# ai4ce/V2X-Sim

Measured on AMD Instinct MI355X. Metric: BEV frames/sec, V2VNet 5-agent detection (256x256 BEV), higher is better.
Workload: dtype bf16

## Files before the change

### v2x-sim_amd/csrc/api.hip

```cpp
#include "common.h"

static thread_local char g_err[512] = "";

void v2x_set_error(const char *fmt, ...) {
    va_list ap;
    va_start(ap, fmt);
    vsnprintf(g_err, sizeof(g_err), fmt, ap);
    va_end(ap);
}

extern "C" __attribute__((weak)) int v2x_probe_build_marker;
extern "C" int v2x_abi_version(void) { return &v2x_probe_build_marker != nullptr ? -V2X_AMD_ABI_VERSION : V2X_AMD_ABI_VERSION; }

#include <atomic>
#include <mutex>
#include <strings.h>
namespace {
struct TuneEntry { const char *name; int def; };
const TuneEntry kTune[V2X_TUNE_COUNT] = {
    {"STREAM_WAVES", 8}, {"STREAM_G", 1}, {"STREAM_WT", 1}, {"STORE_X4", 1}, {"STREAM_PERSIST", 1}, {"STREAM_WIDE", 1},
    {"WIDE3", 1}, {"HALO_PP", 1}, {"VOXELIZE_LDS", 1}, {"WARP_LDS", 2}, {"S2_G", 1}, {"GRU_XCD_WALK", 1}, {"HALO_XCD", 1}, {"WGRAD_TR", 1}, {"BN_PARTIAL_T", 1}, {"WGRAD_REDUCE4", 1}, {"CONV1X1", 1},
};
std::atomic<int> g_tune[V2X_TUNE_COUNT];
std::once_flag g_tune_once;
void tune_init() {
    for (int i = 0; i < V2X_TUNE_COUNT; ++i) {
        char env[64];
        snprintf(env, sizeof(env), "V2X_%s", kTune[i].name);
        const char *e = getenv(env);
        g_tune[i].store((e && *e) ? atoi(e) : kTune[i].def, std::memory_order_relaxed);
    }
}
int tune_find(const char *name) {
    if (!name) return -1;
    if (strncasecmp(name, "V2X_", 4) == 0) name += 4;
    for (int i = 0; i < V2X_TUNE_COUNT; ++i)
        if (strcasecmp(name, kTune[i].name) == 0) return i;
    return -1;
}
}

int v2x_tune(int id) {
    std::call_once(g_tune_once, tune_init);
    return g_tune[id].load(std::memory_order_relaxed);
}
extern "C" int v2x_tuning_set(const char *name, int value) {
    const int i = tune_find(name);
    V2X_REQUIRE(i >= 0, "v2x_tuning_set: unknown switch '%s'", name ? name : "(null)");
    std::call_once(g_tune_once, tune_init);
    g_tune[i].store(value, std::memory_order_relaxed);
    return V2X_OK;
}
extern "C" int v2x_tuning_get(const char *name, int *value) {
    const int i = tune_find(name);
// ... 6 lines not shown
```

### v2x-sim_amd/csrc/common.h

```cpp
#pragma once
#include <hip/hip_runtime.h>
#include <stdint.h>
#include <stdio.h>
#include <stdarg.h>

#include "../../include/v2x_amd.h"

typedef __attribute__((ext_vector_type(8))) __bf16 bf16x8_t;
typedef __attribute__((ext_vector_type(4))) float f32x4_t;
typedef __attribute__((ext_vector_type(16))) float f32x16_t;

void v2x_set_error(const char *fmt, ...);

enum v2x_tune_id {
    V2X_TUNE_STREAM_WAVES,
    V2X_TUNE_STREAM_G,
    V2X_TUNE_STREAM_WT,
    V2X_TUNE_STORE_X4,
    V2X_TUNE_STREAM_PERSIST,
    V2X_TUNE_STREAM_WIDE,
    V2X_TUNE_WIDE3,
    V2X_TUNE_HALO_PP,
    V2X_TUNE_VOXELIZE_LDS,
    V2X_TUNE_WARP_LDS,
    V2X_TUNE_S2_G,
    V2X_TUNE_GRU_XCD_WALK,
    V2X_TUNE_HALO_XCD,
    V2X_TUNE_WGRAD_TR,
    V2X_TUNE_BN_PARTIAL_T,
    V2X_TUNE_WGRAD_REDUCE4,
    V2X_TUNE_CONV1X1,
    V2X_TUNE_COUNT
};
int v2x_tune(int id);

#define V2X_REQUIRE(cond, ...)            \
    do {                                  \
        if (!(cond)) {                    \
            v2x_set_error(__VA_ARGS__);   \
            return V2X_EINVAL;            \
        }                                 \
    } while (0)

#define V2X_CHECK_LAUNCH(name)                                                   \
    do {                                                                         \
        hipError_t e_ = hipGetLastError();                                       \
        if (e_ != hipSuccess) {                                                  \
            v2x_set_error("%s: launch failed: %s", name, hipGetErrorString(e_)); \
            return V2X_EIO;                                                      \
        }                                                                        \
    } while (0)

#define V2X_MAX_DEVICES 32
struct v2x_once_per_device { bool done[V2X_MAX_DEVICES]; };
static inline bool v2x_first_use_on_device(v2x_once_per_device &o) {
    int dev = 0;
    if (hipGetDevice(&dev) != hipSuccess || dev < 0 || dev >= V2X_MAX_DEVICES) return true;
    if (o.done[dev]) return false;
    o.done[dev] = true;
    return true;
}

__device__ __forceinline__ uint16_t f32_to_bf16_rne(float f) {
    uint32_t u = __float_as_uint(f);
// ... 55 lines not shown
```

### v2x-sim_amd/csrc/conv_halo.hip

```cpp
#include "common.h"
#include <cstdlib>

static __device__ __attribute__((aligned(64))) unsigned int g_zero_page_h[16];

typedef const __attribute__((address_space(1))) void *gptr_t;
typedef __attribute__((address_space(3))) void *lptr_t;

__device__ __forceinline__ void glds16h(const void *g, char *lds_wave_base) {
    __builtin_amdgcn_global_load_lds((gptr_t)g, (lptr_t)lds_wave_base, 16, 0, 0);
}

struct HaloArgs {
    const uint16_t *in0;
    const uint16_t *in1;
    const uint32_t *bits;
    int zbits;
    int N, H, W;
    const uint16_t *w;
    const float *scale, *shift;
    int relu;
    void *out;
    int out_cstride, out_coff;
    const uint16_t *w2;
    const float *scale2, *shift2;
// ... 486 lines not shown
                    if constexpr (EPI2 == 2) {
                        const bool second = a.split > 0 && co >= a.split;
                        float *dst = second ? reinterpret_cast<float *>(a.out2) + pix * a.out2_cstride + (co - a.split)
                                            : reinterpret_cast<float *>(a.out) + pix * a.out_cstride + a.out_coff + co;
                        *reinterpret_cast<float4 *>(dst) = make_float4(v0, v1, v2, v3);
                    } else {
                        uint2 o;
                        o.x = pack_bf16x2(v0, v1);
                        o.y = pack_bf16x2(v2, v3);
                        uint16_t *dst = reinterpret_cast<uint16_t *>(a.out) + pix * a.out_cstride + a.out_coff + co;
                        *reinterpret_cast<uint2 *>(dst) = o;
                    }
                }
            }
        }
        if constexpr (DB) {
            cur ^= 1;
        } else {
            __builtin_amdgcn_s_barrier();
        }
    }
}

template <int C0, int C1, int COUT, int COUT2, int EPI2>
__global__ __launch_bounds__(256) __attribute__((amdgpu_waves_per_eu((C0 == 0 && C1 == 64 && COUT2 == 64) ? 1 : 2, 2))) void conv3x3_halo_kernel(const HaloArgs a) {
    conv3x3_halo_body<C0, C1, COUT, COUT2, EPI2, true>(a);
}

template <int C0, int C1, int COUT, int COUT2, int EPI2, bool BITS>
__global__ __launch_bounds__(256) __attribute__((amdgpu_waves_per_eu(4, 4))) void conv3x3_halo_sb_kernel(const HaloArgs a) {
    conv3x3_halo_body<C0, C1, COUT, COUT2, EPI2, false, BITS>(a);
}

template <int C0, int C1, int COUT, int COUT2 = 0>
__global__ __launch_bounds__(512) __attribute__((amdgpu_waves_per_eu(2, 2))) void conv3x3_halo_pp_kernel(const HaloArgs a) {
    constexpr int SPP0 = C0 / 8, SPP1 = C1 / 8;
    constexpr int NS1 = round64(PH * PW * SPP1);
    constexpr int NS0 = C0 ? round64(PH0 * PW0 * SPP0) : 0;
    constexpr int PATCH_BYTES = (NS0 + NS1) * 16;
    constexpr int KSLOTS = 9 * (SPP0 + SPP1);
    constexpr int W_BYTES = KSLOTS * COUT * 16;
    constexpr int TCO = COUT / 16;
    static_assert(C0 % 32 == 0 && C1 % 32 == 0 && (TCO == 2 || TCO == 4), "ping-pong form: 32 or 64 output channels");
    static_assert(W_BYTES % 1024 == 0, "weights are moved 1 KiB per wave instruction");
    constexpr int TCO2 = COUT2 / 16;
    static_assert(COUT2 == 0 || (COUT2 == 64 && COUT == 64), "chained 1x1: 64 -> 64 (conv1_2 -> conv3d_1)");
    constexpr int N_STORES = (COUT2 ? TCO2 : TCO) * 4;

    extern __shared__ __attribute__((aligned(16))) char smem[];
    const uint32_t relu_floor = a.relu ? 0u : 0x80008000u;
    char *s_w = smem;
    char *s_patch = smem + W_BYTES;
    float *s_ss = reinterpret_cast<float *>(smem + W_BYTES + 2 * PATCH_BYTES);
    for (int i = threadIdx.x; i < COUT; i += 512) {
        s_ss[i] = a.scale[i];
        s_ss[COUT + i] = a.shift[i];
    }
    if constexpr (COUT2 > 0) {
        for (int i = threadIdx.x; i < COUT2; i += 512) {
            s_ss[2 * COUT + i] = a.scale2[i];
            s_ss[2 * COUT + COUT2 + i] = a.shift2[i];
        }
    }

    const int tid = threadIdx.x;
    const int lane = tid & 63;
    const int wave = __builtin_amdgcn_readfirstlane(tid >> 6);
    const int grp = wave >> 2, wv = wave & 3;
// ... 279 lines not shown
                    uint32_t ox[2], oy[2];
#pragma unroll
                    for (int h = 0; h < 2; ++h) {
                        ox[h] = v2x_relu_bf16x2_floor(pack_bf16x2(acc[i + h][f][0] * sc[h].x + sf[h].x, acc[i + h][f][1] * sc[h].y + sf[h].y), relu_floor);
                        oy[h] = v2x_relu_bf16x2_floor(pack_bf16x2(acc[i + h][f][2] * sc[h].z + sf[h].z, acc[i + h][f][3] * sc[h].w + sf[h].w), relu_floor);
                    }
                    v2x_store_pair_x4(reinterpret_cast<uint16_t *>(a.out) + ((size_t)(n * a.H + y) * a.W + x) * a.out_cstride + a.out_coff + i * 16 + fq * 4, fq,
                                      ox[0], oy[0], ox[1], oy[1]);
                }
            }
            return;
        }
#pragma unroll
        for (int i = 0; i < TCO; ++i) {
            const int co = i * 16 + fq * 4;
            const float4 sc = *reinterpret_cast<const float4 *>(ss + co);
            const float4 sf = *reinterpret_cast<const float4 *>(ss + COUT + co);
#pragma unroll
            for (int f = 0; f < 4; ++f) {
                const int y = y0 + 2 * wv + (f >> 1), x = x0 + (f & 1) * 16 + fj;
                float v0 = acc[i][f][0] * sc.x + sf.x, v1 = acc[i][f][1] * sc.y + sf.y;
                float v2 = acc[i][f][2] * sc.z + sf.z, v3 = acc[i][f][3] * sc.w + sf.w;
                uint2 o;
                o.x = pack_bf16x2(v0, v1);
                o.y = pack_bf16x2(v2, v3);
                o.x = v2x_relu_bf16x2_floor(o.x, relu_floor);
                o.y = v2x_relu_bf16x2_floor(o.y, relu_floor);
                uint16_t *dst = reinterpret_cast<uint16_t *>(a.out) + ((size_t)(n * a.H + y) * a.W + x) * a.out_cstride + a.out_coff + co;
                *reinterpret_cast<uint2 *>(dst) = o;
            }
        }
    };

    const int n_pairs = a.n_tiles >> 1;
    const v2x_tile_walk walk = v2x_xcd_tile_walk(n_pairs, a.xcd_walk);
    const int K = walk.first < walk.end ? (walk.end - walk.first + walk.step - 1) / walk.step : 0;
    auto tile_of = [&](int k) { return 2 * (walk.first + k * walk.step) + grp; };

    if (grp == 0) load_patch(tile_of(0));
    __syncthreads();

    for (int i = 0; i <= 2 * K; ++i) {
        if ((i & 1) == grp) {
            if ((i >> 1) < K) compute();
        } else {
            const int m = (i - grp - 1) / 2;
            if (m + 1 < K) load_patch(tile_of(m + 1));
            if (m >= 0) {
                epilogue(tile_of(m));
                if constexpr (N_STORES == 8) {
                    if (a.x4) asm volatile("s_waitcnt vmcnt(4)" ::: "memory");
                    else asm volatile("s_waitcnt vmcnt(8)" ::: "memory");
                } else {
                    if (a.x4) asm volatile("s_waitcnt vmcnt(8)" ::: "memory");
                    else asm volatile("s_waitcnt vmcnt(16)" ::: "memory");
                }
            } else {
                asm volatile("s_waitcnt vmcnt(0)" ::: "memory");
            }
        }
        __builtin_amdgcn_sched_barrier(0);
        __builtin_amdgcn_s_barrier();
        __builtin_amdgcn_sched_barrier(0);
    }
    static_assert(N_STORES == 8 || N_STORES == 16, "the counted waits above know 8 or 16 stores per tile and wave");
}

template <int C0, int C1, int COUT, int COUT2 = 0>
static int launch_halo_pp(const HaloArgs &a, hipStream_t s) {
    constexpr int NS1 = round64(PH * PW * (C1 / 8));
    constexpr int NS0 = C0 ? round64(PH0 * PW0 * (C0 / 8)) : 0;
    constexpr int smem = 9 * (C0 + C1) / 8 * COUT * 16 + 2 * (NS0 + NS1) * 16 + 2 * COUT * 4 + 2 * COUT2 * 4;
    static_assert(smem <= 160 * 1024, "LDS budget");
    static v2x_once_per_device attr_once;
    auto kern = &conv3x3_halo_pp_kernel<C0, C1, COUT, COUT2>;
    if (v2x_first_use_on_device(attr_once)) {
        (void)hipFuncSetAttribute(reinterpret_cast<const void *>(kern), hipFuncAttributeMaxDynamicSharedMemorySize, smem);
    }
    int grid = 256;
    if (grid > a.n_tiles / 2) grid = a.n_tiles / 2;
    hipLaunchKernelGGL(kern, dim3(grid), dim3(512), smem, s, a);
    V2X_CHECK_LAUNCH("conv3x3_halo_pp_kernel");
    return V2X_OK;
}

constexpr int PWH = PW / 2;

template <int C0, int C1, int COUT>
__global__ __launch_bounds__(512) __attribute__((amdgpu_waves_per_eu(2, 2))) void conv3x3_halo_ppc_kernel(const HaloArgs a) {
    constexpr int SPP0 = C0 / 8, SPP1 = C1 / 8;
    constexpr int NS1 = round64(2 * PH * PWH * SPP1);
    constexpr int NS0 = round64(PH0 * PW0 * SPP0);
    constexpr int PATCH_BYTES = (NS0 + NS1) * 16;
    constexpr int W_UP_BYTES = 16 * SPP0 * COUT * 16;
    constexpr int W_BYTES = W_UP_BYTES + 9 * SPP1 * COUT * 16;
    constexpr int TCO = COUT / 16;
    constexpr int KC0 = C0 / 32, KC1 = C1 / 32;
    static_assert(C0 % 32 == 0 && C1 % 32 == 0 && C0 > 0 && C1 > 0 && TCO == 2, "parity-class form: two sources, 32 output channels");
    static_assert(W_BYTES % 1024 == 0, "weights are moved 1 KiB per wave instruction");
    constexpr int N_STORES = TCO * 4;

    extern __shared__ __attribute__((aligned(16))) char smem[];
    const uint32_t relu_floor = a.relu ? 0u : 0x80008000u;
    char *s_w = smem;
    char *s_patch = smem + W_BYTES;
    float *s_ss = reinterpret_cast<float *>(smem + W_BYTES + 2 * PATCH_BYTES);
    for (int i = threadIdx.x; i < COUT; i += 512) {
        s_ss[i] = a.scale[i];
        s_ss[COUT + i] = a.shift[i];
    }

    const int tid = threadIdx.x;
    const int lane = tid & 63;
    const int wave = __builtin_amdgcn_readfirstlane(tid >> 6);
    const int grp = wave >> 2, wv = wave & 3;
// ... 277 lines not shown
            const double slack = fmax(1e-3, 4e-7 / (t * (1.0 - t)));
            a.det_margin = (float)fmin(log(t / (1.0 - t)) - slack, 16.0);
        }
    }
    a.det_cap = d->det_cap;
    {
        const int cmax = d->C1 ? (d->C0 > d->C1 ? d->C0 : d->C1) : d->C0;
        if ((long long)(PH * d->W + PW) * cmax >= (1 << 20)) return 1;
    }
    a.tiles_x = d->W / TW;
    a.tiles_y = d->H / TH;
    a.n_tiles = d->N * a.tiles_x * a.tiles_y;
    const int co2 = d->Cout2 > 0 ? (d->Cout2 + 15) / 16 * 16 : 0;
    const int e2 = d->Cout2 > 0 ? (d->epilogue == V2X_EPI_DET ? 3 : (d->epilogue == V2X_EPI_F32 ? 2 : 1)) : 0;
#define HALO_CASE(c0, c1, co, c2, ep) \
    if (C0 == c0 && C1 == c1 && d->Cout == co && co2 == c2 && e2 == ep) return launch_halo<c0, c1, co, c2, ep>(a, s);
    if (C0 == 0 && C1 == 32 && d->Cout == 32 && co2 == 0 && e2 == 0)
        return d->in_format == 1 ? launch_halo_sb<0, 32, 32, 0, 0, true>(a, s) : launch_halo_sb<0, 32, 32, 0, 0, false>(a, s);
    if (d->in_format == 1) return 1;
    if (d->w_layout == 3) {
        if (C0 == 64 && C1 == 32 && d->Cout == 32 && co2 == 0 && e2 == 0) return launch_halo_ppc<64, 32, 32>(a, s);
        return 1;
    }
    if (C0 == 64 && C1 == 32 && d->Cout == 32 && co2 == 0 && e2 == 0 && a.n_tiles >= 2 && a.n_tiles % 2 == 0) {
        if (v2x_tune(V2X_TUNE_HALO_PP) != 0) return launch_halo_pp<64, 32, 32>(a, s);
    }
    HALO_CASE(64, 32, 32, 0, 0)
    if (C0 == 0 && C1 == 64 && d->Cout == 64 && co2 == 0 && e2 == 0 && a.n_tiles >= 2 && a.n_tiles % 2 == 0) {
        if (v2x_tune(V2X_TUNE_HALO_PP) != 0) return launch_halo_pp<0, 64, 64>(a, s);
    }
    HALO_CASE(0, 64, 64, 0, 0)
    if (C0 == 0 && C1 == 64 && d->Cout == 64 && co2 == 64 && e2 == 1 && d->Cout2 == 64 && a.n_tiles >= 2 && a.n_tiles % 2 == 0 &&
        d->split == 0)
        return launch_halo_pp<0, 64, 64, 64>(a, s);
    HALO_CASE(0, 64, 64, 64, 1)
    HALO_CASE(0, 64, 32, 0, 0)
    HALO_CASE(0, 32, 64, 0, 0)
    HALO_CASE(0, 32, 64, 48, 2)
    HALO_CASE(0, 32, 32, 16, 2)
    if (e2 == 3) {
        if (!(C0 == 0 && C1 == 32 && d->Cout == 64 && d->Cout2 == 64 && d->det_counts && d->out && d->out2 && d->det_cap > 0 &&
              d->det_cap <= 4096 && (long long)d->H * d->W * 6 < (1 << 20)))
            return 1;
        return launch_halo<0, 32, 64, 64, 3>(a, s);
    }
#undef HALO_CASE
    return 1;
}
```

### v2x-sim_amd/csrc/conv_stream.hip

```cpp
#include "conv_stream.h"
#include <cstdlib>
#include <type_traits>



#ifndef V2X_STREAM_PSWZ_BUILD
#define V2X_STREAM_PSWZ_BUILD 1
#endif
#define PSWZ(pc) (((pc) >> V2X_STREAM_PSWZ_BUILD) & 3)
#ifndef V2X_STREAM_LSS_BUILD
#define V2X_STREAM_LSS_BUILD 1
#endif

template <int N>
__device__ __forceinline__ void wait_vmcnt() {
    asm volatile("s_waitcnt vmcnt(%0)" ::"n"(N) : "memory");
}

template <int BCO>
constexpr int chain_lds_bytes() { return BCO * BCO * 2 + 2 * BCO * 4; }

template <int BCO, int NT>
__device__ __forceinline__ void stage_chain(const StreamArgs &a, char *cl) {
    constexpr int NKS = BCO / 32;
// ... 424 lines not shown
            f32x4_t g[3];
#pragma unroll
            for (int q = 0; q < 3; ++q) g[q] = (f32x4_t){0.f, 0.f, 0.f, 0.f};
            for (int sp = 0; sp < ksplit; ++sp)
#pragma unroll
                for (int q = 0; q < 3; ++q) g[q] += *reinterpret_cast<const f32x4_t *>(ws + ((size_t)sp * npix + pix) * w_rows + row + 16 * q);
            float h[4];
#pragma unroll
            for (int r = 0; r < 4; ++r) {
                const float4 b = reinterpret_cast<const float4 *>(scale)[c + r];
                h[r] = v2x_gru_h0(g[0][r], g[1][r], g[2][r], b);
            }
            uint2 o;
            o.x = pack_bf16x2(h[0], h[1]);
            o.y = pack_bf16x2(h[2], h[3]);
            *reinterpret_cast<uint2 *>(out + pix * out_cstride + out_coff + c) = o;
        } else {
            f32x4_t v = (f32x4_t){0.f, 0.f, 0.f, 0.f};
            for (int sp = 0; sp < ksplit; ++sp) v += *reinterpret_cast<const f32x4_t *>(ws + ((size_t)sp * npix + pix) * w_rows + c);
            const float4 sc = *reinterpret_cast<const float4 *>(scale + c), sf = *reinterpret_cast<const float4 *>(shift + c);
            uint2 o;
            o.x = pack_bf16x2(v[0] * sc.x + sf.x, v[1] * sc.y + sf.y);
            o.y = pack_bf16x2(v[2] * sc.z + sf.z, v[3] * sc.w + sf.w);
            if (relu) {
                o.x = v2x_relu_bf16x2(o.x);
                o.y = v2x_relu_bf16x2(o.y);
            }
            *reinterpret_cast<uint2 *>(out + pix * out_cstride + out_coff + c) = o;
        }
    }
}


template <int BCO, int EPI>
__global__ __launch_bounds__(512) __attribute__((amdgpu_waves_per_eu(2, 2))) void conv3x3_stream8_kernel(const StreamArgs a) {
    constexpr bool PERSIST = (EPI != SEPI_CHAIN);
    constexpr int TH = 16, TW = 32;
    constexpr int PW = TW + 2, PH = TH + 2, PW0 = TW / 2 + 2, PH0 = TH / 2 + 2;
    constexpr int TCO = BCO / 16;
    constexpr int W_PIECES = BCO / 16;
    constexpr int SLICE_BYTES = BCO * 64;
    constexpr int N_ST = (EPI == SEPI_GRU) ? (TCO / 3) * 4 : TCO * 4;
    static_assert(PH * PW * 4 <= (PATCH8_PIECES - 1) * 64, "patch must leave the last piece as padding");
    static_assert(W_PIECES <= 8, "at most one weight DMA per wave per step");
    static_assert(4 + N_ST <= 63, "vmcnt is a 6-bit counter");

    extern __shared__ __attribute__((aligned(16))) char smem[];
    char *s_ring = smem;
    char *s_patch = smem + RING * SLICE_BYTES;
    char *s_dummy = s_patch + (PATCH8_PIECES - 1) * 1024;

    const int tid = threadIdx.x;
    const int lane = tid & 63;
    const int wave = __builtin_amdgcn_readfirstlane(tid >> 6);
    const int grp = wave >> 2, wv = wave & 3;
    const int fj = lane & 15, fq = lane >> 4;

    const int nwg = gridDim.x;
    int bid = blockIdx.x;
    {
        const int q = nwg >> 3, r = nwg & 7, xcd = bid & 7, i = bid >> 3;
        bid = (xcd < r ? xcd * (q + 1) : r * (q + 1) + (xcd - r) * q) + i;
    }
    const int n_tiles = a.n_px_tiles * a.n_co_tiles;
    const int co_tile = bid % a.n_co_tiles;
    const int txy = a.tiles_x * a.tiles_y;

    const int nc0 = a.C0 >> 5, nchunks = (a.C0 + a.C1) >> 5;
    const int S = nchunks * 9;
    const uint16_t *wbase = a.w + (size_t)co_tile * nchunks * 9 * (BCO * 32);
    const void *zero_page = a.w + (size_t)a.n_co_tiles * nchunks * 9 * (BCO * 32);
    char *s_chain = smem + RING * SLICE_BYTES + 2 * PATCH8_BYTES;
    if constexpr (EPI == SEPI_CHAIN) stage_chain<BCO, 512>(a, s_chain);

    auto tile_coords = [&](int t, int &n, int &y0, int &x0) {
        const int px_tile = t / a.n_co_tiles;
        n = px_tile / txy;
        const int trem = px_tile - n * txy;
        const int ty = trem / a.tiles_x;
        y0 = ty * TH;
        x0 = (trem - ty * a.tiles_x) * TW;
    };
    auto desc = [&](int n, int y0, int x0, int t, bool hf) -> int {
        const int L = (wave + 8 * t) * 64 + lane;
        const int pix = L >> 2, phys = L & 3;
        if (!hf) {
            const int pr = pix / PW, pc = pix - pr * PW;
            const int y = y0 - 1 + pr, x = x0 - 1 + pc;
            const bool ok = pix < PH * PW && (unsigned)y < (unsigned)a.H && (unsigned)x < (unsigned)a.W;
            return ok ? ((((n * a.H + y) * a.W + x) << 5) | ((phys ^ PSWZ(pc)) << 3)) : -1;
        }
        const int Hs = a.H >> 1, Ws = a.W >> 1;
        const int pr = pix / PW0, pc = pix - pr * PW0;
        const int y = (y0 >> 1) - 1 + pr, x = (x0 >> 1) - 1 + pc;
        const bool ok = pix < PH0 * PW0 && (unsigned)y < (unsigned)Hs && (unsigned)x < (unsigned)Ws;
        return ok ? ((((n * Hs + y) * Ws + x) << 5) | ((phys ^ PSWZ(pc)) << 3)) : -1;
    };

    int frow[4], ct[4][3];
#pragma unroll
    for (int f = 0; f < 4; ++f) frow[f] = 8 * grp + 2 * wv + (f >> 1);
    auto build_ct = [&](bool hf) {
#pragma unroll
        for (int f = 0; f < 4; ++f) {
            const int col = (f & 1) * 16 + fj;
#pragma unroll
            for (int kx = 0; kx < 3; ++kx) {
                const int pc = hf ? (((col + kx - 1) >> 1) + 1) : (col + kx);
                ct[f][kx] = ((pc << 2) + (fq ^ PSWZ(pc))) * 16;
            }
        }
    };

    const bool has_w = wave < W_PIECES;
    const uint16_t *wsrc = wbase + lane * 8 + wave * 512;
    auto issue_dummy = [&]() { glds16s(zero_page, s_dummy); };
    auto issue_slice = [&](int slice, int slot, bool real) {
// ... 88 lines not shown
#pragma unroll
                    for (int i = 0; i < TCO; ++i)
                        fa[i] = *reinterpret_cast<const bf16x8_t *>(ws + (fq * BCO + i * 16 + fj) * 16);
                    if (relaxed > 0) {
                        wait_vmcnt<4 + N_ST>();
                        --relaxed;
                    } else {
                        wait_vmcnt<4>();
                    }
                    asm volatile("s_waitcnt lgkmcnt(0)" ::: "memory");
                    __builtin_amdgcn_sched_barrier(0);
                    __builtin_amdgcn_s_barrier();
                    __builtin_amdgcn_sched_barrier(0);
#pragma unroll
                    for (int i = 0; i < TCO; ++i)
#pragma unroll
                        for (int f = 0; f < 4; ++f)
                            acc[i][f] = __builtin_amdgcn_mfma_f32_16x16x32_bf16(fa[i], fb[f], acc[i][f], 0, 0, 0);
                    __builtin_amdgcn_sched_barrier(0);
                    __builtin_amdgcn_s_barrier();
                    __builtin_amdgcn_sched_barrier(0);
                }
            }
        }
        stream_epilogue<BCO, TW, EPI, 4, EPI == SEPI_CHAIN, true, EPI == SEPI_CHAIN>(a, acc, co_tile, n, y0, x0, frow, fj, fq, s_chain, nullptr, 0, a.x4 != 0);
        if (!has_next) break;
        tile = next;
        n = nn;
        y0 = ny0;
        x0 = nx0;
        relaxed = 2;
    }
    if (grp == 0) __builtin_amdgcn_s_barrier();
}

int v2x_conv_stream_pc_launch(const StreamArgs &a, hipStream_t s);

int v2x_num_cus() {
    static int n[V2X_MAX_DEVICES] = {0};
    int dev = 0, v = 0;
    if (hipGetDevice(&dev) != hipSuccess || dev < 0 || dev >= V2X_MAX_DEVICES) return 256;
    if (n[dev] == 0)
        n[dev] = (hipDeviceGetAttribute(&v, hipDeviceAttributeMultiprocessorCount, dev) == hipSuccess && v > 0) ? v : 256;
    return n[dev];
}

#define V2X_STREAM8G_ISSUE_DMAS \
                if (grp == 1) { \
                    const int ahead = st + 2; \
                    const int wslot = slot == 0 ? 2 : slot - 1; \
                    if (ahead < S3) nw = issue_weights(ahead, wslot, wv, 4); \
                    else if (has_next && ahead - S3 < S3) nw = issue_weights(ahead - S3, wslot, wv, 4); \
                } else if (fill && kx < 2) { \
                    const int npieces = hfn ? (PH0 * PW0 * 4 + 63) / 64 : PATCH8_PIECES; \
_Pragma("unroll") \
                    for (int t = 0; t < 5; ++t) { \
                        const int tt = kx * 5 + t; \
                        if (wv + 4 * tt >= npieces) break; \
                        int d = pd[0]; \
_Pragma("unroll") \
                        for (int u = 1; u < 10; ++u) d = (tt == u) ? pd[u] : d; \
                        issue_piece(d, kcn, tt, (gc + 1) & 1); \
                    } \
                }
template <int BCO, int EPI, bool WT = false>
__global__ __launch_bounds__(512) __attribute__((amdgpu_waves_per_eu(2, 2))) void conv3x3_stream8g_kernel(const StreamArgs a) {
// ... 280 lines not shown
        constexpr bool LSS = V2X_STREAM_LSS_BUILD != 0 && EPI != SEPI_GRU;
        if constexpr (WT)
            stream_epilogue<BCO / 2, TW, EPI, 8, false, true, true>(a, acc, co_tile * 2 + coh, n, y0, x0, frow, fj, fq, nullptr,
                                                                    LSS ? (lds_cf_t *)s_ss + coh * (EPI == SEPI_GRU ? 4 * (BCO / 6) : BCO / 2) : (lds_cf_t *)nullptr, BCO, a.x4 != 0);
        else stream_epilogue<BCO, TW, EPI, 4, false, true, true>(a, acc, co_tile, n, y0, x0, frow, fj, fq, nullptr, LSS ? (lds_cf_t *)s_ss : (lds_cf_t *)nullptr, BCO, a.x4 != 0);
        if (!has_next) break;
        tile = next;
        n = nn;
        y0 = ny0;
        x0 = nx0;
        relaxed = true;
    }
    if (grp == 0) __builtin_amdgcn_s_barrier();
}

template <int BCO, int EPI, bool WT = false>
static int launch_stream8g(const StreamArgs &a, hipStream_t s) {
    constexpr int smem = 3 * 3 * BCO * 64 + 2 * PATCH8_BYTES + 1024;
    static_assert(smem <= 160 * 1024, "LDS budget");
    static v2x_once_per_device attr_once;
    auto kern = &conv3x3_stream8g_kernel<BCO, EPI, WT>;
    if (v2x_first_use_on_device(attr_once)) {
        (void)hipFuncSetAttribute(reinterpret_cast<const void *>(kern), hipFuncAttributeMaxDynamicSharedMemorySize, smem);
    }
    const int n_tiles = a.n_px_tiles * a.n_co_tiles;
    int grid = n_tiles;
    int g = v2x_num_cus() / a.n_co_tiles * a.n_co_tiles;
    if (g > 0 && g < n_tiles) grid = g;
    hipLaunchKernelGGL(kern, dim3(grid), dim3(512), smem, s, a);
    V2X_CHECK_LAUNCH("conv3x3_stream8g_kernel");
    return V2X_OK;
}

template <int BCO, int EPI>
static int launch_stream8(const StreamArgs &a, hipStream_t s) {
    constexpr int smem = RING * BCO * 64 + 2 * PATCH8_BYTES + (EPI == SEPI_CHAIN ? chain_lds_bytes<BCO>() : 0);
    static v2x_once_per_device attr_once;
    auto kern = &conv3x3_stream8_kernel<BCO, EPI>;
    if (v2x_first_use_on_device(attr_once)) {
        (void)hipFuncSetAttribute(reinterpret_cast<const void *>(kern), hipFuncAttributeMaxDynamicSharedMemorySize, smem);
    }
    const int n_tiles = a.n_px_tiles * a.n_co_tiles;
    int grid = n_tiles;
    if (v2x_tune(V2X_TUNE_STREAM_PERSIST) != 0) {
        int g = v2x_num_cus() / a.n_co_tiles * a.n_co_tiles;
        if (EPI != SEPI_CHAIN && g > 0 && g < n_tiles && ((a.C0 + a.C1) >> 5) >= 2) grid = g;
    }
    hipLaunchKernelGGL(kern, dim3(grid), dim3(512), smem, s, a);
    V2X_CHECK_LAUNCH("conv3x3_stream8_kernel");
    return V2X_OK;
}

constexpr int WPATCH_PIECES = 39;
constexpr int WPATCH_BYTES = WPATCH_PIECES * 1024;

template <int BCO, int EPI>
__global__ __launch_bounds__(256) __attribute__((amdgpu_waves_per_eu(2, 2))) void conv3x3_wide_kernel(const StreamArgs a) {
    constexpr int TH = 16, TW = 32, NF = 8;
    constexpr int PW = TW + 2, PH = TH + 2, PW0 = TW / 2 + 2, PH0 = TH / 2 + 2;
    constexpr int TCO = BCO / 16;
    constexpr int SLICE_BYTES = BCO * 64;
    constexpr int PPW = (WPATCH_PIECES + 3) / 4;
    static_assert(BCO == 64, "wide form: one 64-row channel tile (1 weight DMA per wave and step)");
    static_assert(PH * PW * 4 <= WPATCH_PIECES * 64, "patch must fit its buffer");

    extern __shared__ __attribute__((aligned(16))) char smem[];
    char *s_ring = smem;
    char *s_patch = smem + RING * SLICE_BYTES;

    const int tid = threadIdx.x;
    const int lane = tid & 63;
    const int wave = __builtin_amdgcn_readfirstlane(tid >> 6);
    const int fj = lane & 15, fq = lane >> 4;

    int bid = blockIdx.x;
    {
        const int nwg = gridDim.x, q = nwg >> 3, r = nwg & 7, xcd = bid & 7, i = bid >> 3;
        bid = (xcd < r ? xcd * (q + 1) : r * (q + 1) + (xcd - r) * q) + i;
    }
    const int co_tile = bid % a.n_co_tiles;
    const int px_tile = bid / a.n_co_tiles;
    const int txy = a.tiles_x * a.tiles_y;
// ... 421 lines not shown
            if (d->W % 64 != 0) return 1;
            a.tiles_x = d->W / 64;
            a.n_co_tiles = 1;
        } else {
            a.n_co_tiles = d->Cout / 128;
        }
        a.n_px_tiles = d->N * a.tiles_x * a.tiles_y;
        return v2x_conv_stream_pc_launch(a, s);
    }
    const bool chain = d->Cout2 > 0;
    if (d->splitk > 1) {
        const int nchunks = (d->C0 + d->C1) >> 5;
        const int per = (nchunks + d->splitk - 1) / d->splitk;
        if (chain || !d->splitk_ws || d->splitk > nchunks || per * (d->splitk - 1) >= nchunks || (rows != 128 && rows != 96 && rows != 64)) return 1;
        if (d->epilogue == V2X_EPI_GRU) return t16 ? launch_stream_splitk<96, 16, 16, SEPI_GRU>(a, s) : launch_stream_splitk<96, 8, 32, SEPI_GRU>(a, s);
        if (rows == 128) return t16 ? launch_stream_splitk<128, 16, 16, SEPI_BF16>(a, s) : launch_stream_splitk<128, 8, 32, SEPI_BF16>(a, s);
        return t16 ? launch_stream_splitk<64, 16, 16, SEPI_BF16>(a, s) : launch_stream_splitk<64, 8, 32, SEPI_BF16>(a, s);
    }
    if (chain) {
        if ((d->Cout != 64 && d->Cout != 128) || d->Cout2 != d->Cout || d->w_rows != d->Cout || d->epilogue != V2X_EPI_BF16 ||
            !d->weight2 || !d->scale2 || !d->shift2)
            return 1;
    }
    const bool few_chain_tiles = chain && (long long)d->N * (d->H / 16) * (d->W / 32) * 4 < 3ll * v2x_num_cus();
    if (!t16 && d->H % 16 == 0 && (rows == 128 || rows == 96) && !few_chain_tiles) {
        if (v2x_tune(V2X_TUNE_STREAM_WAVES) != 4) {
            a.tiles_y = d->H / 16;
            a.n_px_tiles = d->N * a.tiles_x * a.tiles_y;
            const bool grouped = v2x_tune(V2X_TUNE_STREAM_G) != 0 && !chain && a.n_co_tiles <= v2x_num_cus();
            const int wt = v2x_tune(V2X_TUNE_STREAM_WT);
            if (grouped && wt >= 1 && d->epilogue != V2X_EPI_GRU) return launch_stream8g<128, SEPI_BF16, true>(a, s);
            if (grouped && wt >= 2 && d->epilogue == V2X_EPI_GRU) return launch_stream8g<96, SEPI_GRU, true>(a, s);
            if (d->epilogue == V2X_EPI_GRU) return grouped ? launch_stream8g<96, SEPI_GRU>(a, s) : launch_stream8<96, SEPI_GRU>(a, s);
            if (chain) return launch_stream8<128, SEPI_CHAIN>(a, s);
            return grouped ? launch_stream8g<128, SEPI_BF16>(a, s) : launch_stream8<128, SEPI_BF16>(a, s);
        }
    }
    if (!t16 && d->H % 16 == 0 && rows == 64 && d->epilogue == V2X_EPI_BF16 && ((d->C0 + d->C1) >> 5) >= 2) {
        if (v2x_tune(V2X_TUNE_STREAM_WIDE) != 0) {
            a.tiles_y = d->H / 16;
            a.n_px_tiles = d->N * a.tiles_x * a.tiles_y;
            if (!chain && ((d->C0 + d->C1) >> 5) >= 3 && v2x_tune(V2X_TUNE_WIDE3) != 0) return launch_wide3<64>(a, s);
            return chain ? launch_wide<64, SEPI_CHAIN>(a, s) : launch_wide<64, SEPI_BF16>(a, s);
        }
    }
    if (chain) {
        if (d->Cout == 128) return t16 ? launch_stream<128, 16, 16, SEPI_CHAIN>(a, s) : launch_stream<128, 8, 32, SEPI_CHAIN>(a, s);
        return t16 ? launch_stream<64, 16, 16, SEPI_CHAIN>(a, s) : launch_stream<64, 8, 32, SEPI_CHAIN>(a, s);
    }
    if (d->epilogue == V2X_EPI_GRU) return t16 ? launch_stream<96, 16, 16, SEPI_GRU>(a, s) : launch_stream<96, 8, 32, SEPI_GRU>(a, s);
    if (rows == 128) return t16 ? launch_stream<128, 16, 16, SEPI_BF16>(a, s) : launch_stream<128, 8, 32, SEPI_BF16>(a, s);
    return t16 ? launch_stream<64, 16, 16, SEPI_BF16>(a, s) : launch_stream<64, 8, 32, SEPI_BF16>(a, s);
}
```

### v2x-sim_amd/v2x_sim_amd/ops.py

```python
import ctypes as C

import torch

from . import _lib, tuning
from ._lib import ConvDesc, V2X_EPI_BF16, V2X_EPI_F32, V2X_EPI_GRU, V2X_FUSE_MAX, V2X_FUSE_MEAN, V2X_FUSE_WSUM


from . import _launch
from ._launch import _Prof, _dev, _dev_opt, _stream


import threading as _threading

_latency = _threading.local()


class latency_dispatch:

    def __init__(self, target=0):
        self.target = target

    def __enter__(self):
        _latency.depth = getattr(_latency, "depth", 0) + 1
        self.prev, _latency.target = getattr(_latency, "target", 0), self.target
# ... 24 lines not shown


def conv_kernel_name(pc, H=0, W=0, bits=False, N=0):
    if pc.w_layout == 2 and pc.stride == 2:
        if pc.Cout == 64 and pc.C0 == 32:
            return "conv3x3_s2_resident_kernel<64>"
        rows = 128 if pc.Cout % 128 == 0 else 64
        s2g = tuning.get("S2_G")
        if rows == 128 and pc.C0 >= 64 and s2g != 0:
            Ho, Wo = H // 2, W // 2
            g32 = Ho % 8 == 0 and Wo % 32 == 0
            g16 = not g32 and Ho % 16 == 0 and Wo % 16 == 0
            tiles = N * (Ho * Wo // 256) * (pc.Cout // 128)
            if (g32 or g16) and not (latency_launches() and tiles < 4 * torch.cuda.get_device_properties(0).multi_processor_count):
                return "conv3x3_s2g_kernel<%s>" % ("8, 32" if g32 else "16, 16")
        if not (H % 8 == 0 and W % 64 == 0):
            return "conv3x3_s2_stream_kernel<%d, 8, 16>" % rows
        return "conv3x3_s2_stream_kernel<%d, 4, 32>" % rows
    if pc.w_layout == 2:
        rows = _lib.load().v2x_conv_stream_tile_rows(pc.Cout, pc.epilogue)
        th, tw = (8, 32) if W % 32 == 0 else (16, 16)
        epi = 2 if pc.epilogue == V2X_EPI_GRU else (1 if pc.Cout2 else 0)
        if W % 32 == 0 and H % 16 == 0 and rows == 64 and pc.epilogue == V2X_EPI_BF16 and (pc.C0 + pc.C1) >= 64 \
                and tuning.get("STREAM_WIDE") != 0:
            if epi == 0 and (pc.C0 + pc.C1) >= 96 and tuning.get("WIDE3") != 0:
                return "conv3x3_wide3_kernel<64>"
            return "conv3x3_wide_kernel<64, %d>" % epi
        if W % 32 == 0 and H % 16 == 0 and rows in (96, 128) \
                and tuning.get("STREAM_WAVES") != 4:
            if epi != 1 and tuning.get("STREAM_G") != 0:
                wt = tuning.get("STREAM_WT")
                tiled = (wt >= 1 and epi == 0) or (wt >= 2 and epi == 2)
                return "conv3x3_stream8g_kernel<%d, %d, %s>" % (rows, epi, "true" if tiled else "false")
            return "conv3x3_stream8_kernel<%d, %d>" % (rows, epi)
        return "conv3x3_stream_kernel<%d, %d, %d, %d, false>" % (rows, th, tw, epi)
    if pc.w_layout == 4:
        return "conv3x3_stream8q_kernel" if pc.Cout == 64 else "conv3x3_stream8p_kernel"
    if pc.w_layout == 3:
        return "conv3x3_halo_ppc_kernel<%d, %d, %d>" % (pc.C0, pc.C1, pc.Cout)
    if pc.w_layout == 1:
        c0, c1 = (pc.C0, pc.C1) if pc.C1 else (0, pc.C0)
        co2 = (pc.Cout2 + 15) // 16 * 16 if pc.Cout2 else 0
        e2 = 0 if not pc.Cout2 else (2 if pc.epilogue == V2X_EPI_F32 else 1)
        if (c0, c1, pc.Cout, co2) == (0, 32, 32, 0):
            return "conv3x3_halo_sb_kernel<0, 32, 32, 0, 0, %s>" % ("true" if bits else "false")
        if (c0, c1, pc.Cout, co2, e2) == (0, 64, 64, 64, 1):
            return "conv3x3_halo_pp_kernel<0, 64, 64, 64>"
        if (c0, c1, pc.Cout, co2) in ((64, 32, 32, 0), (0, 64, 64, 0)) and tuning.get("HALO_PP") != 0:
            return "conv3x3_halo_pp_kernel<%d, %d, %d, 0>" % (c0, c1, pc.Cout)
        return "conv3x3_halo_kernel<%d, %d, %d, %d, %d>" % (c0, c1, pc.Cout, co2, e2)
    if (pc.ksize == 1 and pc.stride == 1 and not pc.C1 and not pc.Cout2 and pc.epilogue in (V2X_EPI_BF16, V2X_EPI_F32) and pc.C0 % 32 == 0 and pc.C0 <= 128
            and pc.C0 // 32 != 3 and 4 <= pc.Cout <= 128 and pc.Cout % 4 == 0 and (pc.Cout + 15) // 16 in (1, 2, 3, 4, 6, 8) and tuning.get("CONV1X1") != 0):
        ks, ct = pc.C0 // 32, (pc.Cout + 15) // 16
        return "conv1x1_stream_kernel<%d, %d, %s, %d>" % (ks, ct, "true" if pc.epilogue == V2X_EPI_F32 else "false", 2 if ks * ct >= 16 else 4)
    rows = _lib.load().v2x_conv_tile_rows(pc.Cout, pc.epilogue)
    return "conv_igemm_kernel<%d, %d, %d, %d, %d>" % (_CONV_TILES[rows] + (pc.epilogue,))


class VoxelGrid:

    def __init__(self, voxel_size=(0.25, 0.25, 0.4), area_extents=((-32.0, 32.0), (-32.0, 32.0), (-3.0, 2.0))):
        import math
        self.voxel = tuple(float(v) for v in voxel_size)
        self.extents = tuple((float(lo), float(hi)) for lo, hi in area_extents)
        self.dims = tuple(int(math.ceil(hi / v) - 1 - math.floor(lo / v) + 1)
                          for (lo, hi), v in zip(self.extents, self.voxel))
        self._ext = (C.c_double * 6)(*[x for lohi in self.extents for x in lohi])
        self._vox = (C.c_double * 3)(*self.voxel)
        self._dims = (C.c_int32 * 3)(*self.dims)


def voxelize_bits(points, n_pts, grid, out=None):
    lib = _lib.load()
    if points.dim() != 3:
        raise ValueError("points must be (n_clouds, max_pts, stride)")
    n, mp, st = points.shape
    if tuple(n_pts.shape) != (n,):
        raise ValueError("n_pts must hold one count per cloud: expected shape (%d,), got %s" % (n, tuple(n_pts.shape)))
    X, Y, Z = grid.dims
# ... 480 lines not shown
```

### v2x-sim_amd/v2x_sim_amd/tuning.py

```python
import ctypes as C
import os

_HOST_DEFAULTS = {"CONV_PAIR": 1, "TRAIN_HIP": 1, "TRAIN_GRAPH": 1, "TRAIN_HIP_CONV": 0, "SMALL_BATCH": 2, "WARP_HIP": 1, "WARP_XCD": 1, "SEG_FUSE": 1, "TRAIN_PACK_BATCH": 1, "TRAIN_LOSS_HIP": 1, "TRAIN_GATES_HIP": 1, "PARITY_CLASS": 3, "TAIL_FUSE": 1, "TRAIN_HEAD_PACK": 1, "TRAIN_BN_BIAS_ZERO": 1, "TRAIN_UPCAT_CONV": 1, "TRAIN_SPLITK": 480, "TRAIN_V2V_NHWC": 1, "TRAIN_ADAM_HIP": 1, "SPLITK_TARGET": 320}
LIBRARY_SWITCHES = ("STREAM_WAVES", "STREAM_G", "STREAM_WT", "STORE_X4", "STREAM_PERSIST", "STREAM_WIDE", "WIDE3", "HALO_PP",
                    "VOXELIZE_LDS", "WARP_LDS", "S2_G", "GRU_XCD_WALK", "HALO_XCD", "WGRAD_TR", "BN_PARTIAL_T", "WGRAD_REDUCE4", "CONV1X1")


def _env_int(name, default):
    v = os.environ.get("V2X_" + name, "")
    try:
        return int(v) if v != "" else default
    except ValueError:
        return default


_host = {k: _env_int(k, d) for k, d in _HOST_DEFAULTS.items()}


def _norm(name):
    name = name.upper()
    return name[4:] if name.startswith("V2X_") else name


def get(name):
    name = _norm(name)
    if name in _host:
        return _host[name]
    from . import _lib
    out = C.c_int(0)
    _lib.check(_lib.load().v2x_tuning_get(name.encode(), C.byref(out)), "v2x_tuning_get(%s)" % name)
    return out.value


def set(name, value):
    name = _norm(name)
    old = get(name)
    if name in _host:
        _host[name] = int(value)
# ... 5 lines not shown
```

Before: 6327.

## Add chained-layer forms: early second-layer weight loads in halo_pp and persistent stream8 chain

Adds a CHAIN_FORM switch, on by default (value 3), that selects new variants for two chained-conv paths. In the 64->64->64 halo ping-pong kernel, the epilogue now loads the second 1x1 weights into registers first and issues the next patch load alongside them. Counted vmcnt waits then let the weight loads complete while the patch load is still in flight, before the second MFMA runs on the ReLU'd first-layer output. In the stream8 chain kernel, it enables the persistent grid and recomputes lane ids so the chain epilogue can use a persistent tile loop. The old forms stay available behind the switch bits, at the cost of extra register pressure and hand-written asm waits.

Result: no change. 6308 (-0.3%).

```diff
diff --git a/v2x-sim_amd/csrc/api.hip b/v2x-sim_amd/csrc/api.hip
--- a/v2x-sim_amd/csrc/api.hip
+++ b/v2x-sim_amd/csrc/api.hip
@@ -19,7 +19,7 @@
 struct TuneEntry { const char *name; int def; };
 const TuneEntry kTune[V2X_TUNE_COUNT] = {
     {"STREAM_WAVES", 8}, {"STREAM_G", 1}, {"STREAM_WT", 1}, {"STORE_X4", 1}, {"STREAM_PERSIST", 1}, {"STREAM_WIDE", 1},
-    {"WIDE3", 1}, {"HALO_PP", 1}, {"VOXELIZE_LDS", 1}, {"WARP_LDS", 2}, {"S2_G", 1}, {"GRU_XCD_WALK", 1}, {"HALO_XCD", 1}, {"WGRAD_TR", 1}, {"BN_PARTIAL_T", 1}, {"WGRAD_REDUCE4", 1}, {"CONV1X1", 1},
+    {"WIDE3", 1}, {"HALO_PP", 1}, {"VOXELIZE_LDS", 1}, {"WARP_LDS", 2}, {"S2_G", 1}, {"GRU_XCD_WALK", 1}, {"HALO_XCD", 1}, {"WGRAD_TR", 1}, {"BN_PARTIAL_T", 1}, {"WGRAD_REDUCE4", 1}, {"CONV1X1", 1}, {"CHAIN_FORM", 3},
 };
 std::atomic<int> g_tune[V2X_TUNE_COUNT];
 std::once_flag g_tune_once;
diff --git a/v2x-sim_amd/csrc/common.h b/v2x-sim_amd/csrc/common.h
--- a/v2x-sim_amd/csrc/common.h
+++ b/v2x-sim_amd/csrc/common.h
@@ -30,6 +30,7 @@
     V2X_TUNE_BN_PARTIAL_T,
     V2X_TUNE_WGRAD_REDUCE4,
     V2X_TUNE_CONV1X1,
+    V2X_TUNE_CHAIN_FORM,
     V2X_TUNE_COUNT
 };
 int v2x_tune(int id);
diff --git a/v2x-sim_amd/csrc/conv_halo.hip b/v2x-sim_amd/csrc/conv_halo.hip
--- a/v2x-sim_amd/csrc/conv_halo.hip
+++ b/v2x-sim_amd/csrc/conv_halo.hip
@@ -542,8 +542,11 @@
     conv3x3_halo_body<C0, C1, COUT, COUT2, EPI2, false, BITS>(a);
 }
 
-template <int C0, int C1, int COUT, int COUT2 = 0>
-__global__ __launch_bounds__(512) __attribute__((amdgpu_waves_per_eu(2, 2))) void conv3x3_halo_pp_kernel(const HaloArgs a) {
+typedef __attribute__((ext_vector_type(4))) uint32_t u32x4_t;
+
+template <int C0, int C1, int COUT, int COUT2, bool W2FIRST>
+__device__ __forceinline__ void halo_pp_body(const HaloArgs &a) {
+    static_assert(!W2FIRST || (COUT2 == 64 && COUT == 64 && C0 == 0), "W2FIRST is a form of the chained 64 -> 64 -> 64 layer");
     constexpr int SPP0 = C0 / 8, SPP1 = C1 / 8;
     constexpr int NS1 = round64(PH * PW * SPP1);
     constexpr int NS0 = C0 ? round64(PH0 * PW0 * SPP0) : 0;
@@ -889,6 +892,129 @@
         }
     };
 
+    auto store_interval_w2first = [&](int tile, int next) {
+        int ln;
+        asm volatile("v_mbcnt_lo_u32_b32 %0, -1, 0\n\tv_mbcnt_hi_u32_b32 %0, -1, %0" : "=v"(ln));
+        const int fjl = ln & 15, fql = ln >> 4;
+        int zo = 0;
+        asm volatile("" : "+v"(zo));
+        const float *ss = s_ss + zo;
+        constexpr int T2 = TCO2 ? TCO2 : 1;
+        float4 hsc[TCO], hsf[TCO], osc[T2], osf[T2];
+#pragma unroll
+        for (int i = 0; i < TCO; ++i) {
+            const int kappa = 32 * (i >> 1) + 8 * fql + 4 * (i & 1);
+            hsc[i] = *reinterpret_cast<const float4 *>(ss + kappa);
+            hsf[i] = *reinterpret_cast<const float4 *>(ss + COUT + kappa);
+        }
+#pragma unroll
+        for (int i2 = 0; i2 < TCO2; ++i2) {
+            const int co = i2 * 16 + fql * 4;
+            osc[i2] = *reinterpret_cast<const float4 *>(ss + 2 * COUT + co);
+            osf[i2] = *reinterpret_cast<const float4 *>(ss + 2 * COUT + COUT2 + co);
+        }
+        u32x4_t w2r[8];
+        const uint16_t *wlo = a.w2 + (fjl * COUT + fql * 8), *whi = wlo + 32 * COUT;
+#define V2X_W2_LOAD(j, ptr, off) asm volatile("global_load_dwordx4 %0, %1, off offset:" #off : "=&v"(w2r[j]) : "v"(ptr) : "memory")
+        V2X_W2_LOAD(0, wlo, 0);
+        V2X_W2_LOAD(1, wlo, 64);
+        V2X_W2_LOAD(2, wlo, 2048);
+        V2X_W2_LOAD(3, wlo, 2112);
+        V2X_W2_LOAD(4, whi, 0);
+        V2X_W2_LOAD(5, whi, 64);
+        V2X_W2_LOAD(6, whi, 2048);
+        V2X_W2_LOAD(7, whi, 2112);
+#undef V2X_W2_LOAD
+        constexpr int NPMAX = (NS1 + 255) / 256, NPMIN = (NS1 - 192 + 255) / 256;
+        static_assert(NPMAX - NPMIN <= 1 && NPMAX <= 63, "two counted waits cover the four waves of a group");
+        int np = 0;
+        if (next >= 0) {
+            load_patch(next);
+            np = (NS1 - wv * 64 + 255) / 256;
+        }
+        asm volatile("s_cmp_eq_u32 %8, %9\n\t"
+                     "s_cbranch_scc1 1f\n\t"
+                     "s_cmp_eq_u32 %8, %10\n\t"
+                     "s_cbranch_scc1 2f\n\t"
+                     "s_waitcnt vmcnt(0)\n\t"
+                     "s_branch 3f\n"
+                     "1:\n\t"
+                     "s_waitcnt vmcnt(%9)\n\t"
+                     "s_branch 3f\n"
+                     "2:\n\t"
+                     "s_waitcnt vmcnt(%10)\n"
+                     "3:"
+                     : "+v"(w2r[0]), "+v"(w2r[1]), "+v"(w2r[2]), "+v"(w2r[3]), "+v"(w2r[4]), "+v"(w2r[5]), "+v"(w2r[6]), "+v"(w2r[7])
+                     : "s"(np), "n"(NPMAX), "n"(NPMIN)
+                     : "memory", "scc");
+        int n, y0, x0;
+        coords(tile, n, y0, x0);
+        const uint32_t floor2 = a.relu2 ? 0u : 0x80008000u;
+#pragma unroll
+        for (int f = 0; f < 4; ++f) {
+            bf16x8_t hb[COUT / 32];
+#pragma unroll
+            for (int ks = 0; ks < COUT / 32; ++ks) {
+                float h[8];
+#pragma unroll
+                for (int hf = 0; hf < 2; ++hf) {
+                    const int i = 2 * ks + hf;
+                    h[hf * 4 + 0] = acc[i][f][0] * hsc[i].x + hsf[i].x;
+                    h[hf * 4 + 1] = acc[i][f][1] * hsc[i].y + hsf[i].y;
+                    h[hf * 4 + 2] = acc[i][f][2] * hsc[i].z + hsf[i].z;
+                    h[hf * 4 + 3] = acc[i][f][3] * hsc[i].w + hsf[i].w;
+                }
+                uint4 p;
+                p.x = v2x_relu_bf16x2_floor(pack_bf16x2(h[0], h[1]), relu_floor);
+                p.y = v2x_relu_bf16x2_floor(pack_bf16x2(h[2], h[3]), relu_floor);
+                p.z = v2x_relu_bf16x2_floor(pack_bf16x2(h[4], h[5]), relu_floor);
+                p.w = v2x_relu_bf16x2_floor(pack_bf16x2(h[6], h[7]), relu_floor);
+                hb[ks] = __builtin_bit_cast(bf16x8_t, p);
+            }
+            f32x4_t d[T2];
+#pragma unroll
+            for (int i2 = 0; i2 < TCO2; ++i2) d[i2] = (f32x4_t){0.f, 0.f, 0.f, 0.f};
+#pragma unroll
+            for (int ks = 0; ks < COUT / 32; ++ks)
+#pragma unroll
+                for (int i2 = 0; i2 < TCO2; ++i2)
+                    d[i2] = __builtin_amdgcn_mfma_f32_16x16x32_bf16(__builtin_bit_cast(bf16x8_t, w2r[i2 * (COUT / 32) + ks]), hb[ks], d[i2], 0, 0, 0);
+            const int y = y0 + 2 * wv + (f >> 1), x = x0 + (f & 1) * 16 + fjl;
+            uint16_t *prow = reinterpret_cast<uint16_t *>(a.out) + ((size_t)(n * a.H + y) * a.W + x) * a.out_cstride + a.out_coff;
+            if (a.x4) {
+#pragma unroll
+                for (int i2 = 0; i2 + 1 < TCO2; i2 += 2) {
+                    uint32_t ox[2], oy[2];
+#pragma unroll
+                    for (int h = 0; h < 2; ++h) {
+                        const f32x4_t dd = d[i2 + h];
+                        const float4 s2 = osc[i2 + h], t2 = osf[i2 + h];
+                        ox[h] = v2x_relu_bf16x2_floor(pack_bf16x2(dd[0] * s2.x + t2.x, dd[1] * s2.y + t2.y), floor2);
+                        oy[h] = v2x_relu_bf16x2_floor(pack_bf16x2(dd[2] * s2.z + t2.z, dd[3] * s2.w + t2.w), floor2);
+                    }
+                    v2x_store_pair_x4(prow + i2 * 16 + fql * 4, fql, ox[0], oy[0], ox[1], oy[1]);
+                }
+                continue;
+            }
+#pragma unroll
+            for (int i2 = 0; i2 < TCO2; ++i2) {
+                const f32x4_t dd = d[i2];
+                const float4 s2 = osc[i2], t2 = osf[i2];
+                float v0 = dd[0] * s2.x + t2.x, v1 = dd[1] * s2.y + t2.y, v2 = dd[2] * s2.z + t2.z, v3 = dd[3] * s2.w + t2.w;
+                if (a.relu2) {
+                    v0 = fmaxf(v0, 0.f);
+                    v1 = fmaxf(v1, 0.f);
+                    v2 = fmaxf(v2, 0.f);
+                    v3 = fmaxf(v3, 0.f);
+                }
+                uint2 o;
+                o.x = pack_bf16x2(v0, v1);
+                o.y = pack_bf16x2(v2, v3);
+                *reinterpret_cast<uint2 *>(prow + i2 * 16 + fql * 4) = o;
+            }
+        }
+    };
+
     const int n_pairs = a.n_tiles >> 1;
     const v2x_tile_walk walk = v2x_xcd_tile_walk(n_pairs, a.xcd_walk);
     const int K = walk.first < walk.end ? (walk.end - walk.first + walk.step - 1) / walk.step : 0;
@@ -902,9 +1028,12 @@
             if ((i >> 1) < K) compute();
         } else {
             const int m = (i - grp - 1) / 2;
-            if (m + 1 < K) load_patch(tile_of(m + 1));
+            if (!W2FIRST || m < 0) {
+                if (m + 1 < K) load_patch(tile_of(m + 1));
+            }
             if (m >= 0) {
-                epilogue(tile_of(m));
+                if constexpr (W2FIRST) store_interval_w2first(tile_of(m), m + 1 < K ? tile_of(m + 1) : -1);
+                else epilogue(tile_of(m));
                 if constexpr (N_STORES == 8) {
                     if (a.x4) asm volatile("s_waitcnt vmcnt(4)" ::: "memory");
                     else asm volatile("s_waitcnt vmcnt(8)" ::: "memory");
@@ -924,20 +1053,31 @@
 }
 
 template <int C0, int C1, int COUT, int COUT2 = 0>
+__global__ __launch_bounds__(512) __attribute__((amdgpu_waves_per_eu(2, 2))) void conv3x3_halo_pp_kernel(const HaloArgs a) {
+    halo_pp_body<C0, C1, COUT, COUT2, (COUT2 > 0)>(a);
+}
+template <int C0, int C1, int COUT, int COUT2>
+__global__ __launch_bounds__(512) __attribute__((amdgpu_waves_per_eu(2, 2))) void conv3x3_halo_pp_first_kernel(const HaloArgs a) {
+    halo_pp_body<C0, C1, COUT, COUT2, false>(a);
+}
+
+template <int C0, int C1, int COUT, int COUT2 = 0, bool W2FIRST = (COUT2 > 0)>
 static int launch_halo_pp(const HaloArgs &a, hipStream_t s) {
     constexpr int NS1 = round64(PH * PW * (C1 / 8));
     constexpr int NS0 = C0 ? round64(PH0 * PW0 * (C0 / 8)) : 0;
     constexpr int smem = 9 * (C0 + C1) / 8 * COUT * 16 + 2 * (NS0 + NS1) * 16 + 2 * COUT * 4 + 2 * COUT2 * 4;
     static_assert(smem <= 160 * 1024, "LDS budget");
     static v2x_once_per_device attr_once;
-    auto kern = &conv3x3_halo_pp_kernel<C0, C1, COUT, COUT2>;
+    void (*kern)(const HaloArgs);
+    if constexpr (W2FIRST || COUT2 == 0) kern = &conv3x3_halo_pp_kernel<C0, C1, COUT, COUT2>;
+    else kern = &conv3x3_halo_pp_first_kernel<C0, C1, COUT, COUT2>;
     if (v2x_first_use_on_device(attr_once)) {
         (void)hipFuncSetAttribute(reinterpret_cast<const void *>(kern), hipFuncAttributeMaxDynamicSharedMemorySize, smem);
     }
     int grid = 256;
     if (grid > a.n_tiles / 2) grid = a.n_tiles / 2;
     hipLaunchKernelGGL(kern, dim3(grid), dim3(512), smem, s, a);
-    V2X_CHECK_LAUNCH("conv3x3_halo_pp_kernel");
+    V2X_CHECK_LAUNCH(W2FIRST || COUT2 == 0 ? "conv3x3_halo_pp_kernel" : "conv3x3_halo_pp_first_kernel");
     return V2X_OK;
 }
 
@@ -1281,7 +1421,7 @@
     HALO_CASE(0, 64, 64, 0, 0)
     if (C0 == 0 && C1 == 64 && d->Cout == 64 && co2 == 64 && e2 == 1 && d->Cout2 == 64 && a.n_tiles >= 2 && a.n_tiles % 2 == 0 &&
         d->split == 0)
-        return launch_halo_pp<0, 64, 64, 64>(a, s);
+        return (v2x_tune(V2X_TUNE_CHAIN_FORM) & 1) ? launch_halo_pp<0, 64, 64, 64, true>(a, s) : launch_halo_pp<0, 64, 64, 64, false>(a, s);
     HALO_CASE(0, 64, 64, 64, 1)
     HALO_CASE(0, 64, 32, 0, 0)
     HALO_CASE(0, 32, 64, 0, 0)
diff --git a/v2x-sim_amd/csrc/conv_stream.hip b/v2x-sim_amd/csrc/conv_stream.hip
--- a/v2x-sim_amd/csrc/conv_stream.hip
+++ b/v2x-sim_amd/csrc/conv_stream.hip
@@ -480,9 +480,9 @@
 }
 
 
-template <int BCO, int EPI>
-__global__ __launch_bounds__(512) __attribute__((amdgpu_waves_per_eu(2, 2))) void conv3x3_stream8_kernel(const StreamArgs a) {
-    constexpr bool PERSIST = (EPI != SEPI_CHAIN);
+template <int BCO, int EPI, bool CHAIN_PERSIST>
+__device__ __forceinline__ void stream8_body(const StreamArgs &a) {
+    constexpr bool PERSIST = (EPI != SEPI_CHAIN) || CHAIN_PERSIST;
     constexpr int TH = 16, TW = 32;
     constexpr int PW = TW + 2, PH = TH + 2, PW0 = TW / 2 + 2, PH0 = TH / 2 + 2;
     constexpr int TCO = BCO / 16;
@@ -530,7 +530,9 @@
         x0 = (trem - ty * a.tiles_x) * TW;
     };
     auto desc = [&](int n, int y0, int x0, int t, bool hf) -> int {
-        const int L = (wave + 8 * t) * 64 + lane;
+        int ln = lane;
+        if constexpr (EPI == SEPI_CHAIN && CHAIN_PERSIST) asm volatile("v_mbcnt_lo_u32_b32 %0, -1, 0\n\tv_mbcnt_hi_u32_b32 %0, -1, %0" : "=v"(ln));
+        const int L = (wave + 8 * t) * 64 + ln;
         const int pix = L >> 2, phys = L & 3;
         if (!hf) {
             const int pr = pix / PW, pc = pix - pr * PW;
@@ -685,6 +687,15 @@
         relaxed = 2;
     }
     if (grp == 0) __builtin_amdgcn_s_barrier();
+}
+
+template <int BCO, int EPI>
+__global__ __launch_bounds__(512) __attribute__((amdgpu_waves_per_eu(2, 2))) void conv3x3_stream8_kernel(const StreamArgs a) {
+    stream8_body<BCO, EPI, EPI == SEPI_CHAIN>(a);
+}
+template <int BCO>
+__global__ __launch_bounds__(512) __attribute__((amdgpu_waves_per_eu(2, 2))) void conv3x3_stream8_chain1_kernel(const StreamArgs a) {
+    stream8_body<BCO, SEPI_CHAIN, false>(a);
 }
 
 int v2x_conv_stream_pc_launch(const StreamArgs &a, hipStream_t s);
@@ -1031,11 +1042,13 @@
     return V2X_OK;
 }
 
-template <int BCO, int EPI>
+template <int BCO, int EPI, bool CHAIN_PERSIST = (EPI == SEPI_CHAIN)>
 static int launch_stream8(const StreamArgs &a, hipStream_t s) {
     constexpr int smem = RING * BCO * 64 + 2 * PATCH8_BYTES + (EPI == SEPI_CHAIN ? chain_lds_bytes<BCO>() : 0);
     static v2x_once_per_device attr_once;
-    auto kern = &conv3x3_stream8_kernel<BCO, EPI>;
+    void (*kern)(const StreamArgs);
+    if constexpr (EPI != SEPI_CHAIN || CHAIN_PERSIST) kern = &conv3x3_stream8_kernel<BCO, EPI>;
+    else kern = &conv3x3_stream8_chain1_kernel<BCO>;
     if (v2x_first_use_on_device(attr_once)) {
         (void)hipFuncSetAttribute(reinterpret_cast<const void *>(kern), hipFuncAttributeMaxDynamicSharedMemorySize, smem);
     }
@@ -1043,10 +1056,10 @@
     int grid = n_tiles;
     if (v2x_tune(V2X_TUNE_STREAM_PERSIST) != 0) {
         int g = v2x_num_cus() / a.n_co_tiles * a.n_co_tiles;
-        if (EPI != SEPI_CHAIN && g > 0 && g < n_tiles && ((a.C0 + a.C1) >> 5) >= 2) grid = g;
+        if ((EPI != SEPI_CHAIN || CHAIN_PERSIST) && g > 0 && g < n_tiles && ((a.C0 + a.C1) >> 5) >= 2) grid = g;
     }
     hipLaunchKernelGGL(kern, dim3(grid), dim3(512), smem, s, a);
-    V2X_CHECK_LAUNCH("conv3x3_stream8_kernel");
+    V2X_CHECK_LAUNCH((EPI != SEPI_CHAIN || CHAIN_PERSIST) ? "conv3x3_stream8_kernel" : "conv3x3_stream8_chain1_kernel");
     return V2X_OK;
 }
 
@@ -1534,7 +1547,7 @@
             if (grouped && wt >= 1 && d->epilogue != V2X_EPI_GRU) return launch_stream8g<128, SEPI_BF16, true>(a, s);
             if (grouped && wt >= 2 && d->epilogue == V2X_EPI_GRU) return launch_stream8g<96, SEPI_GRU, true>(a, s);
             if (d->epilogue == V2X_EPI_GRU) return grouped ? launch_stream8g<96, SEPI_GRU>(a, s) : launch_stream8<96, SEPI_GRU>(a, s);
-            if (chain) return launch_stream8<128, SEPI_CHAIN>(a, s);
+            if (chain) return (v2x_tune(V2X_TUNE_CHAIN_FORM) & 2) ? launch_stream8<128, SEPI_CHAIN, true>(a, s) : launch_stream8<128, SEPI_CHAIN, false>(a, s);
             return grouped ? launch_stream8g<128, SEPI_BF16>(a, s) : launch_stream8<128, SEPI_BF16>(a, s);
         }
     }
diff --git a/v2x-sim_amd/v2x_sim_amd/ops.py b/v2x-sim_amd/v2x_sim_amd/ops.py
--- a/v2x-sim_amd/v2x_sim_amd/ops.py
+++ b/v2x-sim_amd/v2x_sim_amd/ops.py
@@ -80,6 +80,8 @@
                 wt = tuning.get("STREAM_WT")
                 tiled = (wt >= 1 and epi == 0) or (wt >= 2 and epi == 2)
                 return "conv3x3_stream8g_kernel<%d, %d, %s>" % (rows, epi, "true" if tiled else "false")
+            if epi == 1 and tuning.get("CHAIN_FORM") & 2 == 0:
+                return "conv3x3_stream8_chain1_kernel<%d>" % rows
             return "conv3x3_stream8_kernel<%d, %d>" % (rows, epi)
         return "conv3x3_stream_kernel<%d, %d, %d, %d, false>" % (rows, th, tw, epi)
     if pc.w_layout == 4:
@@ -93,6 +95,8 @@
         if (c0, c1, pc.Cout, co2) == (0, 32, 32, 0):
             return "conv3x3_halo_sb_kernel<0, 32, 32, 0, 0, %s>" % ("true" if bits else "false")
         if (c0, c1, pc.Cout, co2, e2) == (0, 64, 64, 64, 1):
+            if tuning.get("CHAIN_FORM") & 1 == 0:
+                return "conv3x3_halo_pp_first_kernel<0, 64, 64, 64>"
             return "conv3x3_halo_pp_kernel<0, 64, 64, 64>"
         if (c0, c1, pc.Cout, co2) in ((64, 32, 32, 0), (0, 64, 64, 0)) and tuning.get("HALO_PP") != 0:
             return "conv3x3_halo_pp_kernel<%d, %d, %d, 0>" % (c0, c1, pc.Cout)
diff --git a/v2x-sim_amd/v2x_sim_amd/tuning.py b/v2x-sim_amd/v2x_sim_amd/tuning.py
--- a/v2x-sim_amd/v2x_sim_amd/tuning.py
+++ b/v2x-sim_amd/v2x_sim_amd/tuning.py
@@ -3,7 +3,7 @@
 
 _HOST_DEFAULTS = {"CONV_PAIR": 1, "TRAIN_HIP": 1, "TRAIN_GRAPH": 1, "TRAIN_HIP_CONV": 0, "SMALL_BATCH": 2, "WARP_HIP": 1, "WARP_XCD": 1, "SEG_FUSE": 1, "TRAIN_PACK_BATCH": 1, "TRAIN_LOSS_HIP": 1, "TRAIN_GATES_HIP": 1, "PARITY_CLASS": 3, "TAIL_FUSE": 1, "TRAIN_HEAD_PACK": 1, "TRAIN_BN_BIAS_ZERO": 1, "TRAIN_UPCAT_CONV": 1, "TRAIN_SPLITK": 480, "TRAIN_V2V_NHWC": 1, "TRAIN_ADAM_HIP": 1, "SPLITK_TARGET": 320}
 LIBRARY_SWITCHES = ("STREAM_WAVES", "STREAM_G", "STREAM_WT", "STORE_X4", "STREAM_PERSIST", "STREAM_WIDE", "WIDE3", "HALO_PP",
-                    "VOXELIZE_LDS", "WARP_LDS", "S2_G", "GRU_XCD_WALK", "HALO_XCD", "WGRAD_TR", "BN_PARTIAL_T", "WGRAD_REDUCE4", "CONV1X1")
+                    "VOXELIZE_LDS", "WARP_LDS", "S2_G", "GRU_XCD_WALK", "HALO_XCD", "WGRAD_TR", "BN_PARTIAL_T", "WGRAD_REDUCE4", "CONV1X1", "CHAIN_FORM")
 
 
 def _env_int(name, default):
```
